# astra-vision/rain-rendering

Hardware: AMD Instinct MI355X
Metric: rainy frames/sec @ 1242x375, 100 mm/hr (higher is better)
Workload: dtype f64 alpha/mask, f32 colour

## Files before the change

rain-rendering_amd/csrc/rainhip.hip:

```cpp
#include <hip/hip_runtime.h>

#include <dlfcn.h>

#include <cstddef>
#include <cstdio>
#include <cstdlib>
#include <algorithm>
#include <cstring>
#include <string>
#include <type_traits>
#include <mutex>
#include <unordered_map>
#include <vector>

#include "rainhip.h"
#include "rr_device.h"
#include "rr_prepass.h"
#include "rr_deflate.h"
#include "rr_pngrows.h"
#include "rr_jpeg.h"
#include "rr_particles.h"
#include "rr_lens.h"
#include "rr_resize.h"
#include "rr_convert.h"
// ... 2528 lines not shown
    double* hw = sc.wtab + (gi * 2 + axis) * (BR_MAX + 1);
    for (int k = l; k <= r; k += BW_LANES) hw[k] = tab[k] / tot;
  }
}

template <class W>
__device__ inline void blur4(const double* c0, int st, W hw, int r, double& acc0, double& acc1, double& acc2, double& acc3) {
  auto at = [&](int k) { return c0[__mul24(k, st)]; };
  const double wc = hw(r);
  acc0 = c0[0] * wc; acc1 = at(1) * wc; acc2 = at(2) * wc; acc3 = at(3) * wc;
  double a0 = at(-r), a1 = at(1 - r), a2 = at(2 - r), a3 = at(3 - r);
  double b0 = at(r), b1 = at(1 + r), b2 = at(2 + r), b3 = at(3 + r);
  int ii = -r;
  for (; ii + 3 < 0; ii += 4) {
    const double w0 = hw(ii + r), w1 = hw(ii + 1 + r), w2 = hw(ii + 2 + r), w3 = hw(ii + 3 + r);
    const double na0 = at(4 + ii), na1 = at(5 + ii), na2 = at(6 + ii), na3 = at(7 + ii);
    const double nb0 = at(-ii - 1), nb1 = at(-ii - 2), nb2 = at(-ii - 3), nb3 = at(-ii - 4);
    acc0 = acc0 + (a0 + b0) * w0; acc1 = acc1 + (a1 + b1) * w0; acc2 = acc2 + (a2 + b2) * w0; acc3 = acc3 + (a3 + b3) * w0;
    acc0 = acc0 + (a1 + nb0) * w1; acc1 = acc1 + (a2 + b0) * w1; acc2 = acc2 + (a3 + b1) * w1; acc3 = acc3 + (na0 + b2) * w1;
    acc0 = acc0 + (a2 + nb1) * w2; acc1 = acc1 + (a3 + nb0) * w2; acc2 = acc2 + (na0 + b0) * w2; acc3 = acc3 + (na1 + b1) * w2;
    acc0 = acc0 + (a3 + nb2) * w3; acc1 = acc1 + (na0 + nb1) * w3; acc2 = acc2 + (na1 + nb0) * w3; acc3 = acc3 + (na2 + b0) * w3;
    a0 = na0; a1 = na1; a2 = na2; a3 = na3;
    b3 = nb0; b2 = nb1; b1 = nb2; b0 = nb3;
  }
  for (; ii < 0; ii++) {
    const double w = hw(ii + r);
    const double na = at(4 + ii);
    const double nb = at(-ii - 1);
    acc0 = acc0 + (a0 + b0) * w;
    acc1 = acc1 + (a1 + b1) * w;
    acc2 = acc2 + (a2 + b2) * w;
    acc3 = acc3 + (a3 + b3) * w;
    a0 = a1; a1 = a2; a2 = a3; a3 = na;
    b3 = b2; b2 = b1; b1 = b0; b0 = nb;
  }
}

template <int NO, class W>
__device__ inline void blur_n(const double* c0, int st, W hw, int r, double (&acc)[NO]) {
  const double wc = hw(r);
#pragma unroll
  for (int j = 0; j < NO; j++) acc[j] = c0[__mul24(j, st)] * wc;
  for (int ii = -r; ii < 0; ii++) {
    const double w = hw(ii + r);
#pragma unroll
    for (int j = 0; j < NO; j++) acc[j] = acc[j] + (c0[__mul24(j + ii, st)] + c0[__mul24(j - ii, st)]) * w;
  }
}

typedef double double2_a8 __attribute__((ext_vector_type(2), aligned(8)));
__device__ inline void store2(double* o, double a, double b) { *reinterpret_cast<double2_a8*>(o) = double2_a8{a, b}; }

__device__ inline void glds_dword(const void* src, uint32_t lds_byte) {
  uint32_t keep;
  asm volatile("s_mov_b32 %0, m0\n\ts_mov_b32 m0, %2\n\ts_nop 0\n\tglobal_load_lds_dword %1, off\n\ts_mov_b32 m0, %0"
               : "=&s"(keep)
               : "v"(src), "s"(__builtin_amdgcn_readfirstlane((int)lds_byte))
               : "memory");
}
__device__ inline void glds_dwordx4(const void* src, uint32_t lds_byte) {
  uint32_t keep;
  asm volatile("s_mov_b32 %0, m0\n\ts_mov_b32 m0, %2\n\ts_nop 0\n\tglobal_load_lds_dwordx4 %1, off\n\ts_mov_b32 m0, %0"
               : "=&s"(keep)
               : "v"(src), "s"(__builtin_amdgcn_readfirstlane((int)lds_byte))
               : "memory");
}
__global__ __launch_bounds__(256, 4) void k_blur_fused_dma(const FrameDesc* frames, int max_drops, Scratch sc) {
  const int f = blockIdx.y, t = threadIdx.x, lane = t & 63, G = gridDim.x;
  const int wave = __builtin_amdgcn_readfirstlane(t >> 6);
  extern __shared__ __attribute__((aligned(16))) double s_dyn[];
  constexpr int TAB = 2 * (BR_MAX + 1);
  double* tabs = s_dyn;
  double* X = s_dyn + 2 * TAB;
  double* Y = X + sc.blur_bx;
  const uint32_t lds_tabs = (uint32_t)(uintptr_t)(__attribute__((address_space(3))) double*)tabs;
  const uint32_t lds_x = (uint32_t)(uintptr_t)(__attribute__((address_space(3))) double*)X;
  const int n_items = sc.counts[f * 8 + 2];
  if ((int)blockIdx.x >= n_items) return;
  const global_ptr<const uint32_t> items_w = as_global(reinterpret_cast<const uint32_t*>(sc.blur_items + (int64_t)f * max_drops * BLUR_ITEMS_PER_DROP));
  const DropPlan* plans = sc.plan + (int64_t)f * max_drops;
  auto load_item = [&](int item) { return items_w[(int64_t)item * 4 + (lane & 3)]; };
  auto load_plan = [&](int i) { return as_global(reinterpret_cast<const uint32_t*>(plans + i))[lane]; };
  struct PlanView {
    int r1, r2, ew, eh, tw, th, epitch, epad;
    long long a0_off, a1_off;
  };
  auto unpack = [&](uint32_t pv) {
    auto F = [&](size_t byte_off) { return (int)__builtin_amdgcn_readlane((int)pv, (int)(byte_off / 4)); };
    PlanView o;
    o.r1 = F(offsetof(DropPlan, r1)); o.r2 = F(offsetof(DropPlan, r2)); o.ew = F(offsetof(DropPlan, ew)); o.eh = F(offsetof(DropPlan, eh));
    o.tw = F(offsetof(DropPlan, tw)); o.th = F(offsetof(DropPlan, th)); o.epitch = F(offsetof(DropPlan, epitch)); o.epad = F(offsetof(DropPlan, epad));
    o.a0_off = (long long)(((unsigned long long)(unsigned)F(offsetof(DropPlan, a0_off) + 4) << 32) | (unsigned)F(offsetof(DropPlan, a0_off)));
    o.a1_off = (long long)(((unsigned long long)(unsigned)F(offsetof(DropPlan, a1_off) + 4) << 32) | (unsigned)F(offsetof(DropPlan, a1_off)));
    return o;
  };
  auto item_of = [&](uint32_t iv) {
    return make_int4((int)__builtin_amdgcn_readlane((int)iv, 0), (int)__builtin_amdgcn_readlane((int)iv, 1),
                     (int)__builtin_amdgcn_readlane((int)iv, 2), (int)__builtin_amdgcn_readlane((int)iv, 3));
  };
  struct Geo {
    int y0, x0, ho, wo, hop, hi, yp, xa, wd, nx, xs, ys, e_lo, e_hi;
  };
  auto geo = [&](const PlanView& p, int Lwo, int Lho, int st) {
    Geo g;
    const int ntx = (p.ew + Lwo - 1) / Lwo;
    const int sty = st / ntx, stx = st - sty * ntx;
    g.y0 = sty * Lho; g.x0 = stx * Lwo;
    g.ho = imin(Lho, p.eh - g.y0);
    g.wo = imin(Lwo, p.ew - g.x0);
    g.hop = (g.ho + 3) & ~3;
    const int wi = g.wo + 2 * p.r2;
    g.hi = g.hop + 2 * p.r1;
    g.yp = blur_y_pitch(g.wo, p.r2);
    g.xa = imax(0, 2 * p.r2 - g.x0);
    const int xb = imin(wi, p.tw + 2 * p.r2 - g.x0);
    g.wd = imax(xb - g.xa, 0);
    g.nx = g.wd * g.hi;
    g.xs = g.x0 - 2 * p.r2 + g.xa; g.ys = g.y0 - 2 * p.r1;
    const int ra = imin(imax(-g.ys, 0), g.hi), rb = imax(imin(p.th - g.ys, g.hi), ra);
    g.e_lo = ra * g.wd; g.e_hi = rb * g.wd;
    return g;
  };
  auto stage = [&](const PlanView& p, const Geo& g, int drop, bool tables, int tb) {
    if (g.e_hi > g.e_lo && g.wd == p.tw) {
      const char* src = reinterpret_cast<const char*>(sc.arena + p.a0_off + (int64_t)g.ys * p.tw);
      const int a = (g.e_lo + 1) & ~1, b = g.e_hi & ~1;
      for (int e0 = (a & ~511); e0 < b; e0 += 512) {
        const int e = e0 + wave * 128 + 2 * lane;
        if (e >= a && e < b) glds_dwordx4(src + (int64_t)e * 8, lds_x + (uint32_t)(e0 + wave * 128) * 8u);
      }
      if (wave == 0 && (g.e_lo & 1) && lane < 2) glds_dword(src + (int64_t)g.e_lo * 8 + lane * 4, lds_x + (uint32_t)g.e_lo * 8u);
      if (wave == 1 && (g.e_hi & 1) && g.e_hi - 1 >= g.e_lo && lane < 2) glds_dword(src + (int64_t)(g.e_hi - 1) * 8 + lane * 4, lds_x + (uint32_t)(g.e_hi - 1) * 8u);
    } else if (g.e_hi > g.e_lo) {
      const int wdd = imax(g.wd, 1);
      const float inv_wd = 1.0f / (float)wdd;
      const int dq = (int)((128.0f + 0.5f) * inv_wd), dr = 128 - dq * wdd;
      const char* src = reinterpret_cast<const char*>(sc.arena + p.a0_off) + (lane & 1) * 4;
      const int c0 = g.e_lo >> 7, c1 = (g.e_hi + 127) >> 7;
      int e = c0 * 128 + wave * 32 + (lane >> 1);
      int yy = (int)(((float)e + 0.5f) * inv_wd), xc = e - yy * wdd;
      for (int c = c0; c < c1; c++) {
        if (e >= g.e_lo && e < g.e_hi)
          glds_dword(src + (int64_t)((g.ys + yy) * p.tw + (g.xs + xc)) * 8, lds_x + (uint32_t)(c * 128 + wave * 32) * 8u);
        e += 128;
        xc += dr;
        yy += dq;
        if (xc >= wdd) { xc -= wdd; yy += 1; }
      }
    }
    if (tables) {
      const char* wt = reinterpret_cast<const char*>(sc.wtab + ((int64_t)f * max_drops + drop) * TAB);
      if (wave == 3 && lane < TAB / 2) glds_dwordx4(wt + lane * 16, lds_tabs + (uint32_t)(tb * TAB) * 8u);
    }
  };
  uint32_t iv0 = load_item(blockIdx.x);
  uint32_t pv0 = load_plan((int)__builtin_amdgcn_readlane((int)iv0, 0));
  uint32_t iv1 = load_item(imin((int)blockIdx.x + G, n_items - 1));
  uint32_t pv1 = load_plan((int)__builtin_amdgcn_readlane((int)iv1, 0));
  uint32_t iv2 = load_item(imin((int)blockIdx.x + 2 * G, n_items - 1));
  int it = blockIdx.x;
  int4 item = item_of(iv0);
  PlanView p = unpack(pv0);
  int st = item.y, tb = 0;
  Geo g = geo(p, item.w & 0xffff, item.w >> 16, st);
  stage(p, g, item.x, true, tb);
  PH_DECL
  for (;;) {
    const int r1 = p.r1, r2 = p.r2;
    const double* hw1 = tabs + tb * TAB;
    const double* hw2 = hw1 + (BR_MAX + 1);
    {
      const int nz2 = (g.yp * g.hop + 1) >> 1;
      double2* Y2 = reinterpret_cast<double2*>(Y);
      for (int i = t; i < nz2; i += 256) Y2[i] = make_double2(0.0, 0.0);
    }
    asm volatile("s_waitcnt vmcnt(0)" ::: "memory");
    bool has_next = true, new_item = false;
    int4 nitem = item;
    PlanView np = p;
    int nst = st + 1, ntb = tb;
    if (nst >= item.y + item.z) {
      if (it + G < n_items) {
        new_item = true;
        nitem = item_of(iv1);
        np = unpack(pv1);
        nst = nitem.y;
        if (nitem.x != item.x) ntb = tb ^ 1;
      } else {
        has_next = false;
      }
    }
    {
      iv1 = new_item ? iv2 : iv1;
      pv1 = load_plan((int)__builtin_amdgcn_readlane((int)iv1, 0));
      iv2 = load_item(imin(new_item ? it + 3 * G : it + 2 * G, n_items - 1));
    }
    for (int i = t; i < g.e_lo; i += 256) X[i] = 0.0;
    for (int i = g.e_hi + t; i < g.nx; i += 256) X[i] = 0.0;
    PH(0)
    __syncthreads();
    PH(1)
    {
      const int wd = g.wd, nrb = g.hop >> 2, nv = nrb * wd;
      const float inv_wd = 1.0f / (float)imax(wd, 1);
      for (int idx = t; idx < nv; idx += 256) {
        const int rb = (int)(((float)idx + 0.5f) * inv_wd), xq = idx - rb * wd;
        const double* c0 = X + (4 * rb + r1) * wd + xq;
        double acc0, acc1, acc2, acc3;
        blur4(c0, wd, [&](int k) { return hw1[k]; }, r1, acc0, acc1, acc2, acc3);
        double* o = Y + 4 * rb * g.yp + g.xa + xq;
        o[0] = acc0;
        o[g.yp] = acc1;
        o[2 * g.yp] = acc2;
        o[3 * g.yp] = acc3;
      }
    }
    PH(2)
    __syncthreads();
    PH(3)
    Geo ng = g;
    if (has_next) {
      ng = geo(np, nitem.w & 0xffff, nitem.w >> 16, nst);
      stage(np, ng, nitem.x, ntb != tb, ntb);
    }
    PH(6)
    {
      const int ncb = (g.wo + 3) >> 2, nh = ncb * g.ho;
      const float inv_ncb = 1.0f / (float)ncb;
      double* dst = sc.arena + p.a1_off + ((int64_t)g.y0 * p.epitch + p.epad + g.x0);
      for (int idx = t; idx < nh; idx += 256) {
        const int yq = (int)(((float)idx + 0.5f) * inv_ncb), cb = idx - yq * ncb;
        const int xo = 4 * cb;
        const double* c0 = Y + yq * g.yp + xo + r2;
        double acc0, acc1, acc2, acc3;
        if (r2 > 0) {
          blur4(c0, 1, [&](int k) { return hw2[k]; }, r2, acc0, acc1, acc2, acc3);
        } else {
          acc0 = c0[0]; acc1 = c0[1]; acc2 = c0[2]; acc3 = c0[3];
        }
        double* o = dst + ((int64_t)yq * p.epitch + xo);
        if (xo + 3 < g.wo) {
          store2(o, acc0, acc1); store2(o + 2, acc2, acc3);
        } else {
          o[0] = acc0;
          if (xo + 1 < g.wo) o[1] = acc1;
          if (xo + 2 < g.wo) o[2] = acc2;
        }
      }
    }
    PH(4)
    if (!has_next) break;
    __syncthreads();
    PH(5)
    if (new_item) it += G;
    item = nitem; p = np; st = nst; tb = ntb; g = ng;
  }
  PH_FLUSH(3)
}

typedef double double2_v __attribute__((ext_vector_type(2)));
struct SmallItem {
  int li, r1, r2, tw, th, pw, ph, epitch, epad;
  long long a0, a1;
};
__global__ __launch_bounds__(256, 4) void k_blur_small(const FrameDesc* frames, int max_drops, Scratch sc) {
  const int f = blockIdx.y, lane = threadIdx.x & 63;
  const int wave = __builtin_amdgcn_readfirstlane(threadIdx.x >> 6);
  __shared__ __attribute__((aligned(16))) double Xs[4][BS_X], Ys[4][BS_Y];
  double* X = Xs[wave];
  double* Y = Ys[wave];
  const int n_items = sc.counts[f * 8 + 4];
  const global_ptr<const int32_t> list = as_global(sc.list_small + (int64_t)f * max_drops);
  const DropPlan* plans = sc.plan + (int64_t)f * max_drops;
  const int stride = gridDim.x * 4;
  int it = blockIdx.x * 4 + wave;
  if (it >= n_items) return;
  auto load_plan = [&](int li) { return as_global(reinterpret_cast<const uint32_t*>(plans + li))[lane]; };
  auto unpack = [&](uint32_t pv, int li) {
    auto F = [&](size_t byte_off) { return (int)__builtin_amdgcn_readlane((int)pv, (int)(byte_off / 4)); };
    static_assert(offsetof(DropPlan, a1_off) + 8 <= 256, "DropPlan layout");
    SmallItem o;
    o.li = li;
    o.r1 = F(offsetof(DropPlan, r1)); o.r2 = F(offsetof(DropPlan, r2)); o.tw = F(offsetof(DropPlan, tw)); o.th = F(offsetof(DropPlan, th));
    o.pw = F(offsetof(DropPlan, ew)); o.ph = F(offsetof(DropPlan, eh)); o.epitch = F(offsetof(DropPlan, epitch)); o.epad = F(offsetof(DropPlan, epad));
    o.a0 = (long long)(((unsigned long long)(unsigned)F(offsetof(DropPlan, a0_off) + 4) << 32) | (unsigned)F(offsetof(DropPlan, a0_off)));
    o.a1 = (long long)(((unsigned long long)(unsigned)F(offsetof(DropPlan, a1_off) + 4) << 32) | (unsigned)F(offsetof(DropPlan, a1_off)));
    return o;
  };
  double2_v R[4];
  double nw1 = 0.0, nw2 = 0.0;
  auto issue = [&](const SmallItem& d) {
    const global_ptr<const double2_v> raw2 = as_global(reinterpret_cast<const double2_v*>(sc.arena + d.a0));
    const int n = d.tw * d.th;
#pragma unroll
    for (int j = 0; j < 4; j++) {
      const int k2 = lane + 64 * j;
      R[j] = double2_v{0.0, 0.0};
      if (2 * k2 < n) R[j] = raw2[k2];
    }
    const global_ptr<const double> wt = as_global(sc.wtab + ((int64_t)f * max_drops + d.li) * 2 * (BR_MAX + 1));
    nw1 = (lane <= d.r1) ? wt[d.r1 - lane] : 0.0;
    nw2 = (d.r2 > 0 && lane <= d.r2) ? wt[(BR_MAX + 1) + d.r2 - lane] : 0.0;
  };
  PH_DECL
  const int li0 = __builtin_amdgcn_readfirstlane(list[it]);
  SmallItem cur = unpack(load_plan(li0), li0);
  issue(cur);
  bool has_next = it + stride < n_items;
  int li1 = has_next ? __builtin_amdgcn_readfirstlane(list[it + stride]) : li0;
  uint32_t pv_next = load_plan(li1);
  int32_t li2_v = (it + 2 * stride < n_items) ? list[it + 2 * stride] : 0;
  for (;;) {
    const int r1 = cur.r1, r2 = cur.r2, pw = cur.pw, ph = cur.ph, tw = cur.tw, th = cur.th;
    const int php = (ph + 3) & ~3, hi = php + 2 * r1, yp = blur_y_pitch(pw, r2);
    double* tile = sc.arena + cur.a1;
    {
      const int n = tw * th, top = 2 * r1 * tw;
      double2* X2 = reinterpret_cast<double2*>(X);
#pragma unroll
      for (int j = 0; j < 4; j++) {
        const int k2 = lane + 64 * j;
        if (2 * k2 < n) X2[(top >> 1) + k2] = make_double2(R[j].x, 2 * k2 + 1 < n ? R[j].y : 0.0);
      }
      for (int i = lane; i < (top >> 1); i += 64) X2[i] = make_double2(0.0, 0.0);
      const int e0 = (top + n + 1) >> 1, e1 = (tw * hi + 1) >> 1;
      for (int i = e0 + lane; i < e1; i += 64) X2[i] = make_double2(0.0, 0.0);
      const int nz2 = (yp * php + 1) >> 1;
      double2* Y2 = reinterpret_cast<double2*>(Y);
      for (int i = lane; i < nz2; i += 64) Y2[i] = make_double2(0.0, 0.0);
    }
    const double w1 = nw1, w2 = nw2;
    wave_lds_sync();
    PH(0)
    SmallItem nxt = cur;
    if (has_next) {
      nxt = unpack(pv_next, li1);
      issue(nxt);
      if (it + 2 * stride < n_items) {
        li1 = __builtin_amdgcn_readfirstlane(li2_v);
        pv_next = load_plan(li1);
        if (it + 3 * stride < n_items) li2_v = list[it + 3 * stride];
      }
    }
    const float inv_tw = 1.0f / (float)tw;
    const int nv4 = (php >> 2) * tw;
    if (nv4 <= 16) {
      const int idx = lane;
      if (idx < 4 * nv4) {
        const int row = (int)(((float)idx + 0.5f) * inv_tw), x = idx - row * tw;
        double a[1];
        blur_n<1>(X + (__mul24(row + r1, tw) + x), tw, [&](int k) { return readlane_f64(w1, r1 - k); }, r1, a);
        Y[__mul24(row, yp) + 2 * r2 + x] = a[0];
      }
    } else if (nv4 <= 32) {
      const int idx = lane;
      if (idx < 2 * nv4) {
        const int rb = (int)(((float)idx + 0.5f) * inv_tw), x = idx - rb * tw;
        double a[2];
        blur_n<2>(X + (__mul24(2 * rb + r1, tw) + x), tw, [&](int k) { return readlane_f64(w1, r1 - k); }, r1, a);
        double* o = Y + (__mul24(2 * rb, yp) + 2 * r2 + x);
        o[0] = a[0];
        o[yp] = a[1];
      }
    } else {
      const int nv = nv4;
      for (int idx = lane; idx < nv; idx += 64) {
        const int rb = (int)(((float)idx + 0.5f) * inv_tw), x = idx - rb * tw;
        const double* c0 = X + (__mul24(4 * rb + r1, tw) + x);
        double a0, a1, a2, a3;
        blur4(c0, tw, [&](int k) { return readlane_f64(w1, r1 - k); }, r1, a0, a1, a2, a3);
        double* o = Y + (__mul24(4 * rb, yp) + 2 * r2 + x);
        o[0] = a0;
        o[yp] = a1;
        o[2 * yp] = a2;
        o[3 * yp] = a3;
      }
    }
    wave_lds_sync();
    PH(1)
    const int ncb = (pw + 3) >> 2, nh = ncb * ph;
    const int per_row = (r2 > 0 && nh <= 16) ? pw : (r2 > 0 && nh <= 32) ? (pw + 1) >> 1 : ncb;
    const float inv_per_row = 1.0f / (float)per_row;
    if (nh <= 16 && r2 > 0) {
      const int idx = lane;
      if (idx < pw * ph) {
        const int yq = (int)(((float)idx + 0.5f) * inv_per_row), x = idx - yq * pw;
        double a[1];
        blur_n<1>(Y + (__mul24(yq, yp) + x + r2), 1, [&](int k) { return readlane_f64(w2, r2 - k); }, r2, a);
        tile[(int64_t)yq * cur.epitch + cur.epad + x] = a[0];
      }
    } else if (nh <= 32 && r2 > 0) {
      const int idx = lane, nc2 = per_row;
      if (idx < nc2 * ph) {
        const int yq = (int)(((float)idx + 0.5f) * inv_per_row), xo = 2 * (idx - yq * nc2);
        double a[2];
        blur_n<2>(Y + (__mul24(yq, yp) + xo + r2), 1, [&](int k) { return readlane_f64(w2, r2 - k); }, r2, a);
        double* o = tile + (int64_t)yq * cur.epitch + cur.epad + xo;
        if (xo + 1 < pw) {
          store2(o, a[0], a[1]);
        } else {
          o[0] = a[0];
        }
      }
    } else {
      for (int idx = lane; idx < nh; idx += 64) {
        const int yq = (int)(((float)idx + 0.5f) * inv_per_row), xo = 4 * (idx - yq * ncb);
        const double* c0 = Y + (__mul24(yq, yp) + xo + r2);
        double a0, a1, a2, a3;
        if (r2 > 0) {
          blur4(c0, 1, [&](int k) { return readlane_f64(w2, r2 - k); }, r2, a0, a1, a2, a3);
        } else {
          a0 = c0[0]; a1 = c0[1]; a2 = c0[2]; a3 = c0[3];
        }
        double* o = tile + (int64_t)yq * cur.epitch + cur.epad + xo;
        if (xo + 3 < pw) {
          store2(o, a0, a1); store2(o + 2, a2, a3);
        } else {
          o[0] = a0;
          if (xo + 1 < pw) o[1] = a1;
          if (xo + 2 < pw) o[2] = a2;
        }
      }
    }
    wave_lds_sync();
    PH(2)
    if (!has_next) break;
    it += stride;
    cur = nxt;
    has_next = it + stride < n_items;
  }
  PH_FLUSH(2)
}

constexpr int BIG_GROUPS = 64;
constexpr int BIG_ROWS = 16;
constexpr int BIG_COL_LDS = 2048;

template <class F>
__device__ inline void visit_taps(int a0, int a1, int b0, int b1, int r, F f) {
  a0 = imax(a0, -r); a1 = imin(a1, -1);
  b0 = imax(b0, -r); b1 = imin(b1, -1);
  if (a0 > a1) { a0 = b0; a1 = b1; b0 = 0; b1 = -1; }
  if (b0 <= b1 && b0 < a0) { int t = a0; a0 = b0; b0 = t; t = a1; a1 = b1; b1 = t; }
  if (b0 <= b1 && b0 <= a1 + 1) { a1 = imax(a1, b1); b0 = 0; b1 = -1; }
  for (int ii = a0; ii <= a1; ii++) f(ii);
  for (int ii = b0; ii <= b1; ii++) f(ii);
}

constexpr int SLOW_CAP = 256;
__global__ __launch_bounds__(256) void k_blur_big_weights(const FrameDesc* frames, int max_drops, Scratch sc) {
  const int f = blockIdx.y;
  __shared__ double hw[MAX_R + 1];
  const int n_items = imin(sc.counts[f * 8 + 3], SLOW_CAP);
  for (int w = blockIdx.x; w < 2 * n_items; w += gridDim.x) {
    const int it = w >> 1, axis = w & 1;
    const DropPlan& p = sc.plan[(int64_t)f * max_drops + sc.list_slow[(int64_t)f * max_drops + it]];
    const int r = axis ? p.r2 : p.r1;
    __syncthreads();
    if (r > 0) {
      gauss_half_table(axis ? p.sig2 : p.sig1, r, hw);
      double* o = sc.wtab_big + (((int64_t)f * SLOW_CAP + it) * 2 + axis) * (MAX_R + 1);
      for (int k = threadIdx.x; k <= r; k += 256) o[k] = hw[k];
    }
  }
}

template <int AXIS>
__global__ __launch_bounds__(256) void k_blur(const FrameDesc* frames, int max_drops, Scratch sc) {
  const int f = blockIdx.y, t = threadIdx.x;
  __shared__ double hw[MAX_R + 1];
  __shared__ double s_in[BIG_COL_LDS];
  const int n_items = sc.counts[f * 8 + 3];
  int cur = -1;
  for (int w = blockIdx.x; w < n_items * BIG_GROUPS; w += gridDim.x) {
    const int it = w / BIG_GROUPS, g = w - it * BIG_GROUPS;
    const int64_t gi = (int64_t)f * max_drops + sc.list_slow[(int64_t)f * max_drops + it];
    const DropPlan& p = sc.plan[gi];
    const int r = AXIS == 0 ? p.r1 : p.r2;
    const int tw = p.tw, th = p.th, ew = p.ew, eh = p.eh, r1 = p.r1, r2 = p.r2;
    if (AXIS == 0 ? g >= tw : g * BIG_ROWS >= eh) continue;
    const double* raw = sc.arena + p.a0_off;
    double* fin = sc.arena + p.a1_off;
    double* tmp = fin + (((int64_t)p.epitch * eh + 15) & ~15LL);
    __syncthreads();
    if (cur != it) {
      if (r > 0) {
        if (it < SLOW_CAP) {
          const double* wt = sc.wtab_big + (((int64_t)f * SLOW_CAP + it) * 2 + AXIS) * (MAX_R + 1);
          for (int k = t; k <= r; k += 256) hw[k] = wt[k];
          __syncthreads();
        } else {
          gauss_half_table(AXIS == 0 ? p.sig1 : p.sig2, r, hw);
        }
      }
      cur = it;
    }
    if (AXIS == 0) {
      for (int rx = g; rx < tw; rx += BIG_GROUPS) {
        const bool lds = th <= BIG_COL_LDS;
        __syncthreads();
        if (lds)
          for (int k = t; k < th; k += 256) s_in[k] = raw[(int64_t)k * tw + rx];
        __syncthreads();
        auto R = [&](int yy) -> double {
          const int ry = yy - r1;
          return (ry >= 0 && ry < th) ? (lds ? s_in[ry] : raw[(int64_t)ry * tw + rx]) : 0.0;
        };
        for (int y = t; y < eh; y += 256) {
          double acc = R(y) * hw[r];
          visit_taps(r1 - y, r1 - y + th - 1, y - r1 - th + 1, y - r1, r, [&](int ii) { acc = acc + (R(y + ii) + R(y - ii)) * hw[ii + r]; });
          tmp[(int64_t)y * tw + rx] = acc;
        }
      }
    } else {
      for (int y0 = g * BIG_ROWS; y0 < eh; y0 += BIG_GROUPS * BIG_ROWS) {
        const int nr = imin(BIG_ROWS, eh - y0);
        const bool lds = nr * tw <= BIG_COL_LDS;
        __syncthreads();
        if (lds)
          for (int k = t; k < nr * tw; k += 256) s_in[k] = tmp[(int64_t)y0 * tw + k];
        __syncthreads();
        for (int idx = t; idx < nr * ew; idx += 256) {
          const int yy = idx / ew, x = idx - yy * ew;
          auto T = [&](int xx) -> double {
            const int rx = xx - r2;
            return (rx >= 0 && rx < tw) ? (lds ? s_in[yy * tw + rx] : tmp[(int64_t)(y0 + yy) * tw + rx]) : 0.0;
          };
          double acc;
          if (r2 > 0) {
            acc = T(x) * hw[r];
            visit_taps(r2 - x, r2 - x + tw - 1, x - r2 - tw + 1, x - r2, r, [&](int ii) { acc = acc + (T(x + ii) + T(x - ii)) * hw[ii + r]; });
          } else {
            acc = T(x);
          }
          fin[(int64_t)(y0 + yy) * p.epitch + p.epad + x] = acc;
        }
      }
    }
  }
}

__global__ __launch_bounds__(256) void k_bin(const FrameDesc* frames, Dims dm, int max_drops, int ctiles_x, int nct, Scratch sc) {
  const int f = blockIdx.y, ct = blockIdx.x;
  const int cty = ct / ctiles_x, ctx_ = ct - cty * ctiles_x;
  const int t = threadIdx.x, lane = t & 63, wave = t >> 6;
  const int n = frames[f].n_drops;
  const int x0 = ctx_ * CTILE, y0 = cty * CTILE, x1 = min(x0 + CTILE, dm.W), y1 = min(y0 + CTILE, dm.H);
  const int4* bbox = sc.bbox + (int64_t)f * max_drops;
  uint16_t* out = sc.clist + ((int64_t)f * nct + ct) * max_drops;
  __shared__ int s_cnt[4];
  int total = 0;
  for (int base = 0; base < n; base += 256) {
    const int i = base + t;
    bool hit = false;
    if (i < n) {
      const int4 bb = bbox[i];
      hit = bb.x < x1 && bb.z > x0 && bb.y < y1 && bb.w > y0;
    }
    const unsigned long long bal = __ballot(hit);
    if (lane == 0) s_cnt[wave] = __popcll(bal);
    __syncthreads();
    int off = total;
    for (int w = 0; w < 4; w++) {
      const int cw = s_cnt[w];
      if (w < wave) off += cw;
      total += cw;
    }
    if (hit) out[off + __popcll(bal & ((1ull << lane) - 1ull))] = (uint16_t)i;
    __syncthreads();
  }
  if (t == 0) sc.ccount[(int64_t)f * nct + ct] = total;
}

constexpr int BIN_SEG = 8192;
__global__ __launch_bounds__(256) void k_bin_rows(const FrameDesc* frames, Dims dm, int max_drops, int ctiles_x, int nct, Scratch sc) {
  const int f = blockIdx.y, cty = blockIdx.x;
  const int t = threadIdx.x, lane = t & 63, wave = t >> 6;
  const int n = frames[f].n_drops;
  const int y0 = cty * CTILE, y1 = min(y0 + CTILE, dm.H);
  const int4* bbox = sc.bbox + (int64_t)f * max_drops;
  __shared__ uint16_t s_idx[BIN_SEG], s_x0[BIN_SEG], s_x1[BIN_SEG];
  __shared__ int s_cnt[4];
  __shared__ int s_total[64];
  for (int k = t; k < ctiles_x; k += 256) s_total[k] = 0;
  for (int seg = 0; seg < n; seg += BIN_SEG) {
    const int seg_n = min(BIN_SEG, n - seg);
    int m = 0;
    for (int base = 0; base < seg_n; base += 256) {
      const int i = seg + base + t;
      bool hit = false;
      int4 bb = make_int4(0, 0, 0, 0);
      if (base + t < seg_n) {
        bb = bbox[i];
        hit = bb.x < bb.z && bb.y < y1 && bb.w > y0;
      }
      const unsigned long long bal = __ballot(hit);
      if (lane == 0) s_cnt[wave] = __popcll(bal);
      __syncthreads();
      int off = m;
      for (int w = 0; w < 4; w++) {
        const int cw = s_cnt[w];
        if (w < wave) off += cw;
        m += cw;
      }
      if (hit) {
        const int o = off + __popcll(bal & ((1ull << lane) - 1ull));
        s_idx[o] = (uint16_t)i;
        s_x0[o] = (uint16_t)imax(bb.x, 0);
        s_x1[o] = (uint16_t)imin(bb.z, 65535);
      }
      __syncthreads();
    }
    for (int ctx_ = wave; ctx_ < ctiles_x; ctx_ += 4) {
      const int x0 = ctx_ * CTILE, x1 = min(x0 + CTILE, dm.W);
      uint16_t* out = sc.clist + ((int64_t)f * nct + (cty * ctiles_x + ctx_)) * max_drops;
      int total = s_total[ctx_];
      for (int base = 0; base < m; base += 64) {
        const int k = base + lane;
        const bool hit = k < m && (int)s_x0[k] < x1 && (int)s_x1[k] > x0;
        const unsigned long long bal = __ballot(hit);
        if (hit) out[total + __popcll(bal & ((1ull << lane) - 1ull))] = s_idx[k];
        total += __popcll(bal);
      }
      if (lane == 0) s_total[ctx_] = total;
    }
    __syncthreads();
  }
  __syncthreads();
  for (int k = t; k < ctiles_x; k += 256) sc.ccount[(int64_t)f * nct + cty * ctiles_x + k] = s_total[k];
}

__global__ __launch_bounds__(256) void k_pad_visits(const FrameDesc* frames, Dims dm, int max_drops, Scratch sc) {
  const int f = blockIdx.y, i = blockIdx.x * 4 + (threadIdx.x >> 6), lane = threadIdx.x & 63;
  if (i >= frames[f].n_drops) return;
  const int64_t gi = (int64_t)f * max_drops + i;
  if (!sc.blended[gi]) return;
  const DropPlan& p = sc.plan[gi];
  const int4 e = sc.bbox[gi];
  const int w = p.vis_w, n = p.vis_w * p.vis_h;
  const int64_t base = (int64_t)f * dm.H * dm.W;
  for (int k = lane; k < n; k += 64) {
    const int y = p.vis_y0 + k / w, x = p.vis_x0 + k % w;
    if (x < 0 || y < 0 || x >= dm.W || y >= dm.H) continue;
    const bool in_tile = x >= e.x && x < e.z && y >= e.y && y < e.w;
    atomicMin((in_tile ? sc.eff_first : sc.pad_first) + base + (int64_t)y * dm.W + x, i);
  }
}
__device__ inline double clip_unit_np(double v) { return v < 0.0 ? 0.0 : (v > 1.0 ? 1.0 : v); }

__global__ __launch_bounds__(256) void k_composite(const FrameDesc* frames, Dims dm, rr_camera cam, int max_drops, int tiles_x,
                                                   int tiles_y, int ctiles_x, int nct, Scratch sc) {
  const int f = blockIdx.y;
  const int ntiles = tiles_x * tiles_y, per_xcd = (ntiles + 7) / 8;
  const int tile = (int)(blockIdx.x % 8) * per_xcd + (int)(blockIdx.x / 8);
  if (tile >= ntiles) return;
  const int tyi = tile / tiles_x, txi = tile - tyi * tiles_x;
  const int t = threadIdx.x, lane = t & 63, wave = t >> 6;
  const const_ptr<FrameDesc> fr = as_constant(frames + f);
  const void* const fr_bg = fr->bg;
  const void* const fr_rainy = fr->rainy_bg;
  const void* const fr_depth = fr->depth;
  double* const fr_comp = fr->comp_out;
  double* const fr_mask_f64 = fr->mask_f64;
  int32_t* const fr_mask_i32 = fr->mask_i32;
  const int fr_in_types = fr->in_types, fr_depth_f64 = fr->depth_f64;
  const bool same_bg = fr_bg == fr_rainy;
  const int tx0 = txi * TILE, ty0 = tyi * TILE, tx1 = min(tx0 + TILE, dm.W), ty1 = min(ty0 + TILE, dm.H);
  static_assert(TILE == 16, "k_composite: four 8x8 quarters");
  const int px = tx0 + 8 * (wave & 1) + (lane & 7), py = ty0 + 8 * (wave >> 1) + (lane >> 3);
  const bool live = px < dm.W && py < dm.H;
  const int64_t pix = (int64_t)py * dm.W + px;
  double c[3] = {0, 0, 0}, m = 0.0;
  double sum_b = 0.0;
  if (live) {
    load_px3(fr_rainy, rainy_kind(fr_in_types, same_bg), pix, c);
    if (same_bg) {
      sum_b = (c[0] + c[1]) + c[2];
    } else {
      double b[3];
      load_px3(fr_bg, bg_kind(fr_in_types), pix, b);
      sum_b = (b[0] + b[1]) + b[2];
    }
  }
  if (sc.pad_first && live) {
    const int64_t q = (int64_t)f * dm.H * dm.W + pix;
    if (sc.pad_first[q] < sc.eff_first[q])
      for (int k = 0; k < 3; k++) c[k] = clip_unit_np(c[k]);
  }
  double scene = 1.0e300;
  if (fr_depth && live)
    scene = fr_depth_f64 ? as_global((const double*)fr_depth)[pix] : (double)as_global((const float*)fr_depth)[pix];
  const double ex = cam.exposure_s, ex_rcp = 1.0 / ex;
  const bool tame_px = !live || (fabs(c[0]) < 1.0e50 && fabs(c[1]) < 1.0e50 && fabs(c[2]) < 1.0e50);
  const bool slow_wave = __ballot(!tame_px) != 0ull || (__double_as_longlong(ex) & 0xFFFFFFFFFFFFFLL) == 0xFFFFFFFFFFFFFLL ||
                         !(ex > 1.0e-100 && ex < 1.0e100);
  const CompRec* comp = sc.comp + (int64_t)f * max_drops;
  const int4* bbox = sc.bbox + (int64_t)f * max_drops;
  const double* arena = sc.arena;
  const int ct = (ty0 / CTILE) * ctiles_x + (tx0 / CTILE);
  const uint16_t* clist = sc.clist + ((int64_t)f * nct + ct) * max_drops;
  const int n = sc.ccount[(int64_t)f * nct + ct];
  __shared__ int s_list[4][256];
  __shared__ int s_cnt[4][4];
  const int xm = tx0 + 8, ym = ty0 + 8;
  for (int base = 0; base < n; base += 256) {
    const int k = base + t;
    unsigned hitm = 0;
    int i = 0;
    if (k < n) {
      i = clist[k];
      const int4 bb = bbox[i];
      if (bb.x < tx1 && bb.z > tx0 && bb.y < ty1 && bb.w > ty0) {
        const unsigned xl = bb.x < xm, xr = bb.z > xm, yt = bb.y < ym, yb = bb.w > ym;
        hitm = (xl & yt) | ((xr & yt) << 1) | ((xl & yb) << 2) | ((xr & yb) << 3);
      }
    }
    unsigned long long bal[4];
#pragma unroll
    for (int q = 0; q < 4; q++) bal[q] = __ballot((hitm >> q) & 1u);
    if (lane < 4) s_cnt[wave][lane] = __popcll(lane == 0 ? bal[0] : (lane == 1 ? bal[1] : (lane == 2 ? bal[2] : bal[3])));
    __syncthreads();
    int total = 0;
#pragma unroll
    for (int q = 0; q < 4; q++) {
      int off = 0, tq = 0;
      for (int w = 0; w < 4; w++) {
        const int cw = s_cnt[w][q];
        if (w < wave) off += cw;
        tq += cw;
      }
      if ((hitm >> q) & 1u) s_list[q][off + __popcll(bal[q] & ((1ull << lane) - 1ull))] = i;
// ... 5503 lines not shown
```

Baseline: 19660.

## Deepen small-blur software pipeline by staging next tile's X during pass two

Restructures the per-wave small-item blur loop so the next item's input tile is written into the X LDS buffer (with zero padding) after the vertical pass finishes, overlapping with the horizontal pass, and the prefetch of raw data and weights moves one item further ahead. This aims to hide global-load latency and take the X staging off the critical path at the loop head. In exchange it holds more live registers (an extra SmallItem and weights), which may reduce occupancy, and the loop-carried state becomes more complex.

```diff
diff --git a/rain-rendering_amd/csrc/rainhip.hip b/rain-rendering_amd/csrc/rainhip.hip
--- a/rain-rendering_amd/csrc/rainhip.hip
+++ b/rain-rendering_amd/csrc/rainhip.hip
@@ -2854,6 +2854,19 @@
     nw1 = (lane <= d.r1) ? wt[d.r1 - lane] : 0.0;
     nw2 = (d.r2 > 0 && lane <= d.r2) ? wt[(BR_MAX + 1) + d.r2 - lane] : 0.0;
   };
+  auto stage_x = [&](const SmallItem& d) {
+    const int n = d.tw * d.th, top = 2 * d.r1 * d.tw;
+    const int hi_d = ((d.ph + 3) & ~3) + 2 * d.r1;
+    double2* X2 = reinterpret_cast<double2*>(X);
+    for (int i = lane; i < (top >> 1); i += 64) X2[i] = make_double2(0.0, 0.0);
+    const int e0 = (top + n + 1) >> 1, e1 = (d.tw * hi_d + 1) >> 1;
+    for (int i = e0 + lane; i < e1; i += 64) X2[i] = make_double2(0.0, 0.0);
+#pragma unroll
+    for (int j = 0; j < 4; j++) {
+      const int k2 = lane + 64 * j;
+      if (2 * k2 < n) X2[(top >> 1) + k2] = make_double2(R[j].x, 2 * k2 + 1 < n ? R[j].y : 0.0);
+    }
+  };
   PH_DECL
   const int li0 = __builtin_amdgcn_readfirstlane(list[it]);
   SmallItem cur = unpack(load_plan(li0), li0);
@@ -2861,39 +2874,30 @@
   bool has_next = it + stride < n_items;
   int li1 = has_next ? __builtin_amdgcn_readfirstlane(list[it + stride]) : li0;
   uint32_t pv_next = load_plan(li1);
-  int32_t li2_v = (it + 2 * stride < n_items) ? list[it + 2 * stride] : 0;
+  stage_x(cur);
+  double w1 = nw1, w2 = nw2;
+  SmallItem nxt = cur;
+  int32_t li2_v = 0;
+  if (has_next) {
+    nxt = unpack(pv_next, li1);
+    issue(nxt);
+    if (it + 2 * stride < n_items) {
+      li1 = __builtin_amdgcn_readfirstlane(list[it + 2 * stride]);
+      pv_next = load_plan(li1);
+      if (it + 3 * stride < n_items) li2_v = list[it + 3 * stride];
+    }
+  }
   for (;;) {
-    const int r1 = cur.r1, r2 = cur.r2, pw = cur.pw, ph = cur.ph, tw = cur.tw, th = cur.th;
-    const int php = (ph + 3) & ~3, hi = php + 2 * r1, yp = blur_y_pitch(pw, r2);
+    const int r1 = cur.r1, r2 = cur.r2, pw = cur.pw, ph = cur.ph, tw = cur.tw;
+    const int php = (ph + 3) & ~3, yp = blur_y_pitch(pw, r2);
     double* tile = sc.arena + cur.a1;
     {
-      const int n = tw * th, top = 2 * r1 * tw;
-      double2* X2 = reinterpret_cast<double2*>(X);
-#pragma unroll
-      for (int j = 0; j < 4; j++) {
-        const int k2 = lane + 64 * j;
-        if (2 * k2 < n) X2[(top >> 1) + k2] = make_double2(R[j].x, 2 * k2 + 1 < n ? R[j].y : 0.0);
-      }
-      for (int i = lane; i < (top >> 1); i += 64) X2[i] = make_double2(0.0, 0.0);
-      const int e0 = (top + n + 1) >> 1, e1 = (tw * hi + 1) >> 1;
-      for (int i = e0 + lane; i < e1; i += 64) X2[i] = make_double2(0.0, 0.0);
       const int nz2 = (yp * php + 1) >> 1;
       double2* Y2 = reinterpret_cast<double2*>(Y);
       for (int i = lane; i < nz2; i += 64) Y2[i] = make_double2(0.0, 0.0);
     }
-    const double w1 = nw1, w2 = nw2;
     wave_lds_sync();
     PH(0)
-    SmallItem nxt = cur;
-    if (has_next) {
-      nxt = unpack(pv_next, li1);
-      issue(nxt);
-      if (it + 2 * stride < n_items) {
-        li1 = __builtin_amdgcn_readfirstlane(li2_v);
-        pv_next = load_plan(li1);
-        if (it + 3 * stride < n_items) li2_v = list[it + 3 * stride];
-      }
-    }
     const float inv_tw = 1.0f / (float)tw;
     const int nv4 = (php >> 2) * tw;
     if (nv4 <= 16) {
@@ -2930,6 +2934,24 @@
     }
     wave_lds_sync();
     PH(1)
+    SmallItem aft = nxt;
+    double w2n = w2;
+    if (has_next) {
+      stage_x(nxt);
+      w1 = nw1;
+      w2n = nw2;
+      asm volatile("" : "+v"(w1), "+v"(w2n));
+      if (it + 2 * stride < n_items) {
+        aft = unpack(pv_next, li1);
+        issue(aft);
+        if (it + 3 * stride < n_items) {
+          li1 = __builtin_amdgcn_readfirstlane(li2_v);
+          pv_next = load_plan(li1);
+          if (it + 4 * stride < n_items) li2_v = list[it + 4 * stride];
+        }
+      }
+    }
+    PH(0)
     const int ncb = (pw + 3) >> 2, nh = ncb * ph;
     const int per_row = (r2 > 0 && nh <= 16) ? pw : (r2 > 0 && nh <= 32) ? (pw + 1) >> 1 : ncb;
     const float inv_per_row = 1.0f / (float)per_row;
@@ -2979,6 +3001,8 @@
     if (!has_next) break;
     it += stride;
     cur = nxt;
+    nxt = aft;
+    w2 = w2n;
     has_next = it + stride < n_items;
   }
   PH_FLUSH(2)
```

After: 19700 (median of 5 runs). No clear change (+0.2%).
